# gsalzer/mythril

Hardware: AMD Instinct MI355X
Metric: constraint-candidate evals/sec + % z3 queries discharged on-GPU (higher is better)
Workload: dtype u32 (256-bit as 8x32-bit limbs)

## Files before the change

### mythril_amd/csrc/u256.h

```cpp
#pragma once
#include <math.h>
#include <stdint.h>

#define PF_INL __device__ __forceinline__

#include "u256_cols.h"

namespace pf {

struct u256 {
    uint32_t l[8];
};

PF_INL u256 zero256() {
    u256 r;
#pragma unroll
    for (int i = 0; i < 8; i++) r.l[i] = 0;
    return r;
}

PF_INL u256 ones256() {
    u256 r;
#pragma unroll
    for (int i = 0; i < 8; i++) r.l[i] = 0xffffffffu;
    return r;
}

PF_INL u256 add256(const u256& a, const u256& b) {
    u256 r;
    uint32_t c = 0;
#pragma unroll
    for (int i = 0; i < 8; i++) {
        uint32_t co;
        r.l[i] = __builtin_addc(a.l[i], b.l[i], c, &co);
        c = co;
    }
    return r;
}

PF_INL u256 add256c(const u256& a, const u256& b, uint32_t* cout) {
    u256 r;
    uint32_t c = 0;
#pragma unroll
    for (int i = 0; i < 8; i++) {
        uint32_t co;
        r.l[i] = __builtin_addc(a.l[i], b.l[i], c, &co);
        c = co;
    }
    *cout = c;
    return r;
}

PF_INL u256 sub256(const u256& a, const u256& b) {
    u256 r;
    uint32_t c = 0;
#pragma unroll
    for (int i = 0; i < 8; i++) {
        uint32_t co;
        r.l[i] = __builtin_subc(a.l[i], b.l[i], c, &co);
        c = co;
    }
    return r;
}

PF_INL u256 sub256b(const u256& a, const u256& b, uint32_t* bout) {
    u256 r;
    uint32_t c = 0;
#pragma unroll
    for (int i = 0; i < 8; i++) {
        uint32_t co;
        r.l[i] = __builtin_subc(a.l[i], b.l[i], c, &co);
        c = co;
    }
    *bout = c;
    return r;
}

PF_INL uint32_t ult256(const u256& a, const u256& b) {
    uint32_t c = 0;
#pragma unroll
    for (int i = 0; i < 8; i++) {
        uint32_t co;
        (void)__builtin_subc(a.l[i], b.l[i], c, &co);
        c = co;
    }
    return c;
}

PF_INL uint32_t eq256(const u256& a, const u256& b) {
    uint32_t d = 0;
#pragma unroll
    for (int i = 0; i < 8; i++) d |= a.l[i] ^ b.l[i];
    return d == 0;
}

PF_INL uint32_t iszero256(const u256& a) {
    uint32_t d = 0;
#pragma unroll
    for (int i = 0; i < 8; i++) d |= a.l[i];
    return d == 0;
}

PF_INL u256 neg256(const u256& a) { return sub256(zero256(), a); }

PF_INL u256 not256(const u256& a) {
    u256 r;
#pragma unroll
    for (int i = 0; i < 8; i++) r.l[i] = ~a.l[i];
    return r;
}

PF_INL uint32_t lane_mask(uint32_t c) {
    uint32_t m = 0u - (uint32_t)(c != 0u);
#ifndef PF_HOST_MAC
    asm volatile("" : "+v"(m));
#endif
    return m;
}

PF_INL uint32_t zero_limb() {
    uint32_t z = 0u;
#ifndef PF_HOST_MAC
    asm("" : "+v"(z));
#endif
    return z;
}

PF_INL u256 sel256(uint32_t c, const u256& a, const u256& b) {
    const uint32_t m = lane_mask(c);
    u256 r;
#pragma unroll
    for (int i = 0; i < 8; i++) r.l[i] = (a.l[i] & m) | (b.l[i] & ~m);
    return r;
}

#ifndef PF_HOST_MAC
PF_INL uint32_t wave_max_u32(uint32_t v) {
#pragma unroll
    for (int o = 32; o >= 1; o >>= 1) v = max(v, (uint32_t)__shfl_xor((int)v, o));
    return __builtin_amdgcn_readfirstlane(v);
}
PF_INL uint64_t wave_mask(bool p) { return __builtin_amdgcn_ballot_w64(p); }
#else
PF_INL uint32_t wave_max_u32(uint32_t v) { return v; }
PF_INL uint64_t wave_mask(bool p) { return p ? 1ull : 0ull; }
#endif
PF_INL bool wave_any(uint64_t m) { return m != 0ull; }
PF_INL bool wave_none(uint64_t m) { return m == 0ull; }

PF_INL uint64_t wave_mask_ult256(const u256& a, const u256& b) {
#ifndef PF_HOST_MAC
    uint64_t m;
    uint32_t t;
    asm("v_sub_co_u32 %1, vcc, %2, %10\n\ts_nop 1\n\t"
        "v_subb_co_u32 %1, vcc, %3, %11, vcc\n\ts_nop 1\n\t"
        "v_subb_co_u32 %1, vcc, %4, %12, vcc\n\ts_nop 1\n\t"
        "v_subb_co_u32 %1, vcc, %5, %13, vcc\n\ts_nop 1\n\t"
        "v_subb_co_u32 %1, vcc, %6, %14, vcc\n\ts_nop 1\n\t"
        "v_subb_co_u32 %1, vcc, %7, %15, vcc\n\ts_nop 1\n\t"
        "v_subb_co_u32 %1, vcc, %8, %16, vcc\n\ts_nop 1\n\t"
        "v_subb_co_u32 %1, %0, %9, %17, vcc"
        : "=s"(m), "=&v"(t)
        : "v"(a.l[0]), "v"(a.l[1]), "v"(a.l[2]), "v"(a.l[3]), "v"(a.l[4]), "v"(a.l[5]), "v"(a.l[6]),
          "v"(a.l[7]), "v"(b.l[0]), "v"(b.l[1]), "v"(b.l[2]), "v"(b.l[3]), "v"(b.l[4]), "v"(b.l[5]),
          "v"(b.l[6]), "v"(b.l[7])
        : "vcc");
    return m;
#else
    return wave_mask(ult256(a, b) != 0u);
#endif
}

PF_INL uint32_t sat_u32(double x) {
#ifndef PF_HOST_MAC
    uint32_t r;
    asm("v_cvt_u32_f64 %0, %1" : "=v"(r) : "v"(x));
    return r;
#else
    return (uint32_t)fmin(x, 4294967295.0);
#endif
}

#define PF_COL_NEXT(k)                                   \
    r.l[k] = (uint32_t)acc;                              \
    acc = (acc >> 32) | ((uint64_t)hi << 32);

PF_INL u256 mul256(const u256& a, const u256& b) {
    const uint32_t *x = a.l, *y = b.l;
    u256 r;
    uint64_t acc = 0;
    uint32_t hi = 0;
    col64_1(acc, x[0], y[0]);
    PF_COL_NEXT(0)
    col96_2(acc, hi, x[0], x[1], y[1], y[0]);
    PF_COL_NEXT(1)
    col96_3(acc, hi, x[0], x[1], x[2], y[2], y[1], y[0]);
    PF_COL_NEXT(2)
    col96_4(acc, hi, x[0], x[1], x[2], x[3], y[3], y[2], y[1], y[0]);
    PF_COL_NEXT(3)
    col96_5(acc, hi, x[0], x[1], x[2], x[3], x[4], y[4], y[3], y[2], y[1], y[0]);
    PF_COL_NEXT(4)
    col96_6(acc, hi, x[0], x[1], x[2], x[3], x[4], x[5], y[5], y[4], y[3], y[2], y[1], y[0]);
    PF_COL_NEXT(5)
    col64_7(acc, x[0], x[1], x[2], x[3], x[4], x[5], x[6], y[6], y[5], y[4], y[3], y[2], y[1], y[0]);
    r.l[6] = (uint32_t)acc;
    acc >>= 32;
    col64_8(acc, x[0], x[1], x[2], x[3], x[4], x[5], x[6], x[7], y[7], y[6], y[5], y[4], y[3], y[2], y[1], y[0]);
    r.l[7] = (uint32_t)acc;
    return r;
}

PF_INL u256 sqr256(const u256& a) {
    const uint32_t* x = a.l;
    u256 r;
    r.l[0] = 0u;
    uint64_t acc = 0;
    uint32_t hi = 0;
    col64_1(acc, x[0], x[1]);
    PF_COL_NEXT(1)
    col96_1(acc, hi, x[0], x[2]);
    PF_COL_NEXT(2)
    col96_2(acc, hi, x[0], x[1], x[3], x[2]);
    PF_COL_NEXT(3)
    col96_2(acc, hi, x[0], x[1], x[4], x[3]);
    PF_COL_NEXT(4)
    col96_3(acc, hi, x[0], x[1], x[2], x[5], x[4], x[3]);
    PF_COL_NEXT(5)
    col64_3(acc, x[0], x[1], x[2], x[6], x[5], x[4]);
    r.l[6] = (uint32_t)acc;
    acc >>= 32;
    col64_4(acc, x[0], x[1], x[2], x[3], x[7], x[6], x[5], x[4]);
    r.l[7] = (uint32_t)acc;
    u256 c;
#pragma unroll
    for (int i = 7; i >= 1; i--) c.l[i] = (r.l[i] << 1) | (r.l[i - 1] >> 31);
    c.l[0] = 0u;
    u256 d;
#pragma unroll
    for (int i = 0; i < 4; i++) {
        uint64_t q = 0;
        col64_1(q, x[i], x[i]);
        d.l[2 * i] = (uint32_t)q;
        d.l[2 * i + 1] = (uint32_t)(q >> 32);
    }
    return add256(c, d);
}
#undef PF_COL_NEXT

PF_INL uint32_t mul256_overflows(const u256& a, const u256& b) {
    uint32_t hi = 0;
    u256 r = zero256();
#pragma unroll
    for (int i = 0; i < 8; i++) {
        uint64_t carry = 0;
#pragma unroll
        for (int j = 0; j < 8; j++) {
            if (i + j < 8) {
                uint64_t t = (uint64_t)a.l[i] * b.l[j] + r.l[i + j] + carry;
                r.l[i + j] = (uint32_t)t;
                carry = t >> 32;
            } else {
                hi |= (a.l[i] != 0u && b.l[j] != 0u) ? 1u : 0u;
            }
        }
        hi |= (carry != 0) ? 1u : 0u;
    }
    return hi;
}

PF_INL u256 shl256(const u256& a, uint32_t s, uint32_t big) {
    u256 x = a;
    if (__builtin_expect(1, 1)) {
        uint32_t m = (s >> 7) & 1;
#pragma unroll
        for (int i = 7; i >= 0; i--) x.l[i] = m ? (i >= 4 ? x.l[i - 4] : 0u) : x.l[i];
        m = (s >> 6) & 1;
#pragma unroll
        for (int i = 7; i >= 0; i--) x.l[i] = m ? (i >= 2 ? x.l[i - 2] : 0u) : x.l[i];
        m = (s >> 5) & 1;
#pragma unroll
        for (int i = 7; i >= 0; i--) x.l[i] = m ? (i >= 1 ? x.l[i - 1] : 0u) : x.l[i];
    }
    uint32_t bs = s & 31;
    u256 r;
#pragma unroll
    for (int i = 7; i >= 1; i--) r.l[i] = bs ? ((x.l[i] << bs) | (x.l[i - 1] >> (32 - bs))) : x.l[i];
    r.l[0] = x.l[0] << bs;
    return sel256(big, zero256(), r);
}

PF_INL u256 shr256(const u256& a, uint32_t s, uint32_t f) {
    u256 x = a;
    uint32_t m = (s >> 7) & 1;
#pragma unroll
    for (int i = 0; i < 8; i++) x.l[i] = m ? (i + 4 < 8 ? x.l[i + 4] : f) : x.l[i];
    m = (s >> 6) & 1;
#pragma unroll
    for (int i = 0; i < 8; i++) x.l[i] = m ? (i + 2 < 8 ? x.l[i + 2] : f) : x.l[i];
    m = (s >> 5) & 1;
#pragma unroll
    for (int i = 0; i < 8; i++) x.l[i] = m ? (i + 1 < 8 ? x.l[i + 1] : f) : x.l[i];
    uint32_t bs = s & 31;
    u256 r;
#pragma unroll
    for (int i = 0; i < 7; i++) r.l[i] = bs ? ((x.l[i] >> bs) | (x.l[i + 1] << (32 - bs))) : x.l[i];
    r.l[7] = bs ? ((x.l[7] >> bs) | (f << (32 - bs))) : x.l[7];
    return r;
}

PF_INL uint32_t clz256(const u256& a) {
    uint32_t n = 0, done = 0;
#pragma unroll
    for (int i = 7; i >= 0; i--) {
        uint32_t z = a.l[i] ? (uint32_t)__builtin_clz(a.l[i]) : 32u;
        n += done ? 0u : z;
        done |= (a.l[i] != 0u);
    }
    return n;
}

PF_INL double rcp_f64(double x) {
#ifndef PF_HOST_MAC
    double r = __builtin_amdgcn_rcp(x);
    double e = fma(-x, r, 1.0);
    r = fma(r, e, r);
    e = fma(-x, r, 1.0);
    return fma(r, e, r);
#else
    return 1.0 / x;
#endif
}

PF_INL double to_f64(const u256& a) {
    double d = 0.0;
#pragma unroll
    for (int i = 7; i >= 0; i--) d = fma(d, 4294967296.0, (double)a.l[i]);
    return d;
}

#define PF_DIV_BIAS 0x1p-12
PF_INL void udivrem256(const u256& a, const u256& b, u256* q, u256* r) {
    const uint32_t bz = iszero256(b);
    const uint64_t m_bz = wave_mask(bz != 0u);
#ifndef PF_DIV_FORCE_GENERAL
    if (wave_none(wave_mask(true) & ~(wave_mask_ult256(a, b) | m_bz))) {
        *q = sel256(bz, ones256(), zero256());
        *r = a;
        return;
    }
    if (wave_none(wave_mask((b.l[1] | b.l[2] | b.l[3] | b.l[4] | b.l[5] | b.l[6] | b.l[7]) != 0u))) {
        const uint32_t d = bz ? 1u : b.l[0];
        const double rd = rcp_f64((double)d);
        uint32_t rem = 0;
        u256 Q;
#pragma unroll
        for (int j = 7; j >= 0; j--) {
            const uint64_t num = ((uint64_t)rem << 32) | a.l[j];
            const double dn = (double)rem * 4294967296.0 + (double)a.l[j];
            uint32_t qj = sat_u32(fma(dn, rd, 0x1p-12));
            int64_t rr = (int64_t)(num - (uint64_t)qj * d);
            const uint32_t lo = (uint32_t)(rr < 0);
            qj -= lo;
            rr += (int64_t)(d & lane_mask(lo));
            Q.l[j] = qj;
            rem = (uint32_t)rr;
        }
        u256 R = zero256();
        R.l[0] = rem;
        *q = sel256(bz, ones256(), Q);
        *r = sel256(bz, a, R);
        return;
    }
#endif
    const double rcp = rcp_f64(fmax(to_f64(b), 1.0));
#ifndef PF_DIV_FORCE_GENERAL
    const double qest = fma(to_f64(a), rcp, PF_DIV_BIAS);
    if (wave_none(wave_mask(qest >= 4294967294.0) & ~m_bz)) {
        uint32_t qh = sat_u32(qest);
        u256 R, Q = zero256();
        uint32_t carry = 0, bw = 0;
#pragma unroll
        for (int i = 0; i < 8; i++) {
            const uint64_t p = (uint64_t)qh * b.l[i] + carry;
            carry = (uint32_t)(p >> 32);
            uint32_t bo;
            R.l[i] = __builtin_subc(a.l[i], (uint32_t)p, bw, &bo);
            bw = bo;
        }
        uint32_t bo8;
        const uint32_t r8 = __builtin_subc(zero_limb(), carry, bw, &bo8);
        if (wave_any(wave_mask(r8 != 0u))) {
            const uint32_t neg = (uint32_t)(r8 != 0u);
            const uint32_t m = lane_mask(neg);
            uint32_t c = 0;
#pragma unroll
            for (int i = 0; i < 8; i++) {
                uint32_t co;
                R.l[i] = __builtin_addc(R.l[i], b.l[i] & m, c, &co);
                c = co;
            }
            qh -= neg;
        }
        Q.l[0] = qh;
        *q = sel256(bz, ones256(), Q);
        *r = R;
        return;
    }
#endif
    uint32_t u[9];
#pragma unroll
    for (int i = 0; i < 8; i++) u[i] = a.l[i];
    u256 Q = zero256();
    u[8] = zero_limb();
    uint32_t sfx[9];
    sfx[8] = 0u;
#pragma unroll
    for (int k = 7; k >= 0; k--) sfx[k] = sfx[k + 1] | b.l[k];
#pragma unroll
    for (int j = 7; j >= 0; j--) {
        const uint32_t bhigh = j >= 2 ? sfx[9 - j] : 0u;
        double dr = (double)u[7];
#pragma unroll
        for (int i = 6; i >= j; i--) dr = fma(dr, 4294967296.0, (double)u[i]);
        const double qe = fma(dr, rcp, PF_DIV_BIAS);
        if (wave_none(wave_mask(qe >= 1.0) & ~(m_bz | wave_mask(bhigh != 0u)))) continue;
        const uint32_t skip = bz | (uint32_t)(bhigh != 0u);
        uint32_t q = sat_u32(qe) & ~lane_mask(skip);
        uint64_t carry = 0;
        uint32_t borrow = 0;
#pragma unroll
        for (int i = 0; i + j <= 8; i++) {
            const uint64_t p = (uint64_t)q * (i < 8 ? b.l[i] : 0u) + carry;
            carry = p >> 32;
            uint32_t bo;
            u[j + i] = __builtin_subc(u[j + i], (uint32_t)p, borrow, &bo);
            borrow = bo;
        }
        if (wave_any(wave_mask(u[8] != 0u))) {
            const uint32_t neg = (uint32_t)(u[8] != 0u);
            const uint32_t m = 0u - neg;
            q -= neg;
            uint32_t c = 0;
#pragma unroll
            for (int i = 0; i + j <= 8; i++) {
                uint32_t co;
                u[j + i] = __builtin_addc(u[j + i], (i < 8 ? b.l[i] : 0u) & m, c, &co);
                c = co;
            }
        }
        Q.l[j] = q;
    }
    u256 R;
#pragma unroll
    for (int i = 0; i < 8; i++) R.l[i] = u[i];
    *q = sel256(bz, ones256(), Q);
    *r = R;
}

PF_INL void tbl_put(uint2* tbl, uint32_t stride, uint32_t j, const u256& v) {
#pragma unroll
    for (int p = 0; p < 4; p++) tbl[(j * 4u + p) * stride] = make_uint2(v.l[2 * p], v.l[2 * p + 1]);
}
PF_INL u256 tbl_get(const uint2* tbl, uint32_t stride, uint32_t j) {
    u256 v;
#pragma unroll
    for (int p = 0; p < 4; p++) {
        const uint2 q = tbl[(j * 4u + p) * stride];
        v.l[2 * p] = q.x;
        v.l[2 * p + 1] = q.y;
    }
    return v;
}

template <int WB = 3>
PF_INL u256 exp256(const u256& base, const u256& e, uint32_t nbits, uint2* tbl, uint32_t stride) {
    static_assert(WB >= 1 && WB <= 3, "window");
    constexpr uint32_t NT = 1u << WB;
    u256 r = zero256();
    r.l[0] = 1u;
    if (nbits == 0u) return r;
    tbl_put(tbl, stride, 0u, r);
    tbl_put(tbl, stride, 1u, base);
    if constexpr (WB == 2) {
        const u256 b2 = sqr256(base);
        tbl_put(tbl, stride, 2u, b2);
        tbl_put(tbl, stride, 3u, mul256(b2, base));
    } else {
#pragma unroll 1
        for (uint32_t j = 2; j < NT; j++) {
            const u256 f = tbl_get(tbl, stride, (j & 1u) ? j - 1u : j >> 1);
            const u256 g = (j & 1u) ? base : f;
            tbl_put(tbl, stride, j, mul256(f, g));
        }
    }
    const uint32_t nd = (nbits + WB - 1u) / WB;
    const uint32_t rest = WB * (nd - 1u);
    r = tbl_get(tbl, stride, shr256(e, rest, 0u).l[0] & (NT - 1u));
    u256 ex = shl256(e, (256u - rest) & 255u, 0u);
#pragma unroll 1
    for (uint32_t i = 1; i < nd; i++) {
#pragma unroll 1
        for (int k = 0; k < WB; k++) r = sqr256(r);
        const uint32_t d = ex.l[7] >> (32 - WB);
#pragma unroll
        for (int k = 7; k >= 1; k--) ex.l[k] = (ex.l[k] << WB) | (ex.l[k - 1] >> (32 - WB));
        ex.l[0] <<= WB;
        r = mul256(r, tbl_get(tbl, stride, d));
    }
    return r;
}

template <int WB = 2>
PF_INL u256 exp256_w32(const u256& base, uint32_t e, uint32_t nbits, bool want_b2, uint2* tbl, uint32_t stride) {
    static_assert(WB == 2, "window");
    u256 one = zero256();
    one.l[0] = 1u;
    const bool loop = nbits > 1u;
    if (loop || want_b2) {
        const u256 b2 = sqr256(base);
        tbl_put(tbl, stride, 2u, b2);
        if (loop) {
            tbl_put(tbl, stride, 1u, base);
            tbl_put(tbl, stride, 3u, mul256(b2, base));
        }
    }
    if (!loop) return sel256((uint32_t)(e == 0u), one, base);
    const uint32_t nd = (nbits + WB - 1u) / WB;
    uint32_t d = (e >> (WB * (nd - 1u))) & 3u;
    u256 r = sel256((uint32_t)(d == 0u), one, tbl_get(tbl, stride, d));
#pragma unroll 1
    for (uint32_t i = nd - 1u; i-- > 0u;) {
#pragma unroll 1
        for (int k = 0; k < WB; k++) r = sqr256(r);
        d = (e >> (WB * i)) & 3u;
        r = mul256(r, sel256((uint32_t)(d == 0u), one, tbl_get(tbl, stride, d)));
    }
    return r;
}

#ifndef PF_EXP_SPLIT
#define PF_EXP_SPLIT 8
#endif
#define PF_EXP_WINDOW (PF_EXP_SPLIT <= 20 ? 2 : 3)
#define PF_EXP_TBL_ENTRIES (1 << PF_EXP_WINDOW)

PF_INL uint32_t funnel(uint32_t hi, uint32_t lo, uint32_t s) {
    return (uint32_t)((((uint64_t)hi << 32) | lo) >> s);
}

template <int L>
PF_INL void tsqr(const uint32_t* a, uint32_t* out) {
    uint32_t r[L];
#pragma unroll
    for (int i = 0; i < L; i++) r[i] = 0u;
#pragma unroll
    for (int i = 0; 2 * i + 1 < L; i++) {
        uint64_t c = 0;
#pragma unroll
        for (int j = i + 1; i + j < L; j++) {
            c = (uint64_t)a[i] * a[j] + (uint64_t)r[i + j] + (c >> 32);
            r[i + j] = (uint32_t)c;
        }
    }
#pragma unroll
    for (int i = L - 1; i >= 1; i--) r[i] = funnel(r[i], r[i - 1], 31u);
    r[0] <<= 1;
    uint32_t d[L];
#pragma unroll
    for (int i = 0; 2 * i < L; i++) {
        const uint64_t q = (uint64_t)a[i] * a[i];
        d[2 * i] = (uint32_t)q;
        if (2 * i + 1 < L) d[2 * i + 1] = (uint32_t)(q >> 32);
    }
    uint32_t c = 0;
#pragma unroll
    for (int i = 0; i < L; i++) {
        uint32_t co;
        out[i] = __builtin_addc(r[i], d[i], c, &co);
        c = co;
    }
}

template <int TL, uint32_t TM, int Q>
PF_INL void t_steps(uint32_t* t, uint32_t k0, uint32_t k1) {
    constexpr int L = TL - Q;
#pragma unroll 1
    for (uint32_t k = k0; k < k1; k++) {
        uint32_t sq[L];
        if constexpr (L == 8) {
            u256 a;
#pragma unroll
            for (int i = 0; i < 8; i++) a.l[i] = t[i];
            const u256 s = sqr256(a);
#pragma unroll
            for (int i = 0; i < 8; i++) sq[i] = s.l[i];
        } else {
            tsqr<L>(t, sq);
        }
        const uint32_t sh = 32u - (k + 1u - 32u * Q);
        uint32_t c = 0;
#pragma unroll
        for (int i = Q; i < TL; i++) {
            const uint32_t lo = i > Q ? sq[i > Q ? i - Q - 1 : 0] : 0u;
            uint32_t co;
            t[i] = __builtin_addc(t[i], funnel(sq[i - Q], lo, sh), c, &co);
            c = co;
        }
        t[TL - 1] &= TM;
    }
}


constexpr int v2c(int i) { return (i & 1) ? 0 : 1 + v2c(i >> 1); }
constexpr int v2fact(int j) { return j <= 1 ? 0 : v2c(j) + v2fact(j - 1); }
constexpr int exp_terms(int m) {
    int j = 1;
    while ((j + 1) * (m + 2) - v2fact(j + 1) < 256) j++;
    return j;
}
constexpr int prefix_val(int m, int i) { return (i - 1) * (m + 2) - v2fact(i - 1); }

struct k256 {
    uint32_t l[8];
};
constexpr k256 k_small(uint32_t v) {
    k256 r{};
    r.l[0] = v;
    return r;
}
constexpr k256 k_mul(const k256& a, const k256& b) {
    k256 r{};
    for (int i = 0; i < 8; i++) {
        uint64_t c = 0;
        for (int j = 0; i + j < 8; j++) {
            c = (uint64_t)a.l[i] * b.l[j] + r.l[i + j] + (c >> 32);
            r.l[i + j] = (uint32_t)c;
        }
    }
    return r;
}
constexpr k256 k_inv(const k256& o) {
    k256 x = o;
    for (int it = 0; it < 7; it++) {
        const k256 ox = k_mul(o, x);
        k256 two_minus{};
        uint64_t bw = 0;
        for (int i = 0; i < 8; i++) {
            const uint64_t d = (uint64_t)(i == 0 ? 2u : 0u) - ox.l[i] - bw;
            two_minus.l[i] = (uint32_t)d;
            bw = (d >> 32) & 1u;
        }
        x = k_mul(x, two_minus);
    }
    return x;
}
constexpr k256 exp_oddprod(int i, int j) {
    k256 r = k_small(1u);
    for (int k = i; k <= j; k++) r = k_mul(r, k_small((uint32_t)(k >> v2c(k))));
    return r;
}
constexpr k256 exp_addend(int i, int j, int limbs) {
    k256 r = k_mul(exp_oddprod(i, j), k_inv(exp_oddprod(1, j)));
    for (int k = limbs; k < 8; k++) r.l[k] = 0u;
    return r;
}

template <int L, int LY, uint32_t K0, uint32_t K1, uint32_t K2, uint32_t K3, uint32_t K4, uint32_t K5, uint32_t K6>
PF_INL u256 tmul_add(const u256& a, const u256& b, const k256& k) {
    if constexpr (L >= 8) {
        u256 kk;
#pragma unroll
        for (int i = 0; i < 8; i++) kk.l[i] = k.l[i];
        return add256(mul256(a, b), kk);
    } else {
        u256 r = zero256();
        tmulk<L, LY, K0, K1, K2, K3, K4, K5, K6>(a.l, b.l, r.l);
        return r;
    }
}

template <int L>
PF_INL u256 tmul(const u256& a, const u256& b) {
    if constexpr (L >= 8)
        return mul256(a, b);
    else
        return tmul_add<L, L, 0u, 0u, 0u, 0u, 0u, 0u, 0u>(a, b, k256{});
}

template <int L>
PF_INL u256 sub_mul_small(const u256& a, const u256& b, uint32_t c) {
    u256 r = zero256();
    uint32_t carry = 0, bw = 0;
#pragma unroll
    for (int i = 0; i < L; i++) {
        const uint64_t p = (uint64_t)b.l[i] * c + carry;
        carry = (uint32_t)(p >> 32);
        uint32_t bo;
        r.l[i] = __builtin_subc(a.l[i], (uint32_t)p, bw, &bo);
        bw = bo;
    }
    return r;
}

template <int S, int L>
PF_INL u256 shl_const(const u256& a) {
    constexpr int LS = S / 32, BS = S % 32;
    u256 r = zero256();
#pragma unroll
    for (int i = LS; i < L; i++) {
        const uint32_t hi = a.l[i - LS];
        const uint32_t lo = i - LS - 1 >= 0 ? a.l[i - LS - 1 >= 0 ? i - LS - 1 : 0] : 0u;
        r.l[i] = BS ? funnel(hi, lo, 32 - BS) : hi;
    }
    return r;
}

template <int M, int I, int J>
PF_INL u256 horner(u256& g, const u256& tt) {
    constexpr int S = M + 2 - v2c(I);
    constexpr int P = 256 - prefix_val(M, I);
    constexpr int L = (P + 31) / 32;
    constexpr k256 K = exp_addend(I, J, L);
    constexpr int LY = (I == J || (P - S + 31) / 32 >= L || L == 1) ? L : L - 1;
    u256 inner = zero256();
    if constexpr (I < J) {
        inner = horner<M, I + 1, J>(g, tt);
        g = add256(g, tt);
    } else {
        constexpr k256 C = exp_addend(J + 1, J, L);
#pragma unroll
        for (int i = 0; i < L; i++) inner.l[i] = C.l[i];
    }
    return tmul_add<L, LY, K.l[0], K.l[1], K.l[2], K.l[3], K.l[4], K.l[5], K.l[6]>(shl_const<S, L>(g), inner, K);
}

PF_INL u256 exp256_split(const u256& base, const u256& e, uint2* tbl, uint32_t stride,
                         uint64_t* pt = nullptr) {
#if defined(PF_PROFILE_UNITS) && !defined(PF_HOST_MAC)
#define PF_EXP_STAMP(k)                                        \
    if (pt) {                                                  \
        const uint64_t t_ = __builtin_amdgcn_s_memtime();      \
        pt[k] += t_ - t_last;                                  \
        t_last = t_;                                           \
    }
    uint64_t t_last = __builtin_amdgcn_s_memtime();
#else
#define PF_EXP_STAMP(k)
    (void)pt;
#endif
    constexpr int M = PF_EXP_SPLIT;
    static_assert(M >= 8 && M <= 84, "split");
    constexpr int T = 254 - M;
    constexpr int TL = (T + 31) / 32;
    constexpr uint32_t TM = (T % 32) ? ((1u << (T % 32)) - 1u) : 0xffffffffu;
    constexpr int TB = (T + 3 + 31) / 32;
    constexpr int J = exp_terms(M);
    constexpr int WB = PF_EXP_WINDOW;
    const uint32_t odd = base.l[0] & 1u;
    const uint32_t e_big =
        (e.l[0] >= 256u) | ((e.l[1] | e.l[2] | e.l[3] | e.l[4] | e.l[5] | e.l[6] | e.l[7]) != 0u);
    u256 e0;
#pragma unroll
    for (int i = 0; i < 8; i++)
        e0.l[i] = 32 * i + 32 <= M ? e.l[i] : (32 * i < M ? e.l[i] & ((1u << (M % 32)) - 1u) : 0u);
    const uint32_t nb0 = wave_max_u32(256u - clz256(e0));
    u256 n = shr256(e, (uint32_t)M, 0u);
#pragma unroll
    for (int i = 0; i < 8; i++) n.l[i] = i < TL - 1 ? n.l[i] : (i == TL - 1 ? n.l[i] & TM : 0u);
    const bool series = wave_any(wave_mask(odd != 0u) & ~wave_mask(iszero256(n) != 0u));
    u256 r;
    if constexpr (M <= 32 && WB == 2)
        r = exp256_w32<WB>(base, e0.l[0], nb0 < (uint32_t)M ? nb0 : (uint32_t)M, series && TB == 8, tbl, stride);
    else
        r = exp256<WB>(base, e0, nb0 < (uint32_t)M ? nb0 : (uint32_t)M, tbl, stride);
    PF_EXP_STAMP(0)
    if (series) {
        tbl_put(tbl, stride, 1u, r);
        uint32_t t[TL];
        {
            uint32_t sq[TB];
            if constexpr (M <= 32 && WB == 2 && TB == 8) {
                const u256 b2 = tbl_get(tbl, stride, 2u);
#pragma unroll
                for (int i = 0; i < TB; i++) sq[i] = b2.l[i];
            } else {
                tsqr<TB>(base.l, sq);
            }
            sq[0] -= 1u;
#pragma unroll
            for (int i = 0; i < TL; i++) t[i] = funnel(i + 1 < TB ? sq[i + 1 < TB ? i + 1 : 0] : 0u, sq[i], 3u);
            t[TL - 1] &= TM;
        }
        t_steps<TL, TM, 0>(t, 1u, M < 32 ? (uint32_t)M : 32u);
        if (M > 32) t_steps<TL, TM, 1>(t, 32u, M < 64 ? (uint32_t)M : 64u);
        if (M > 64) t_steps<TL, TM, 2>(t, 64u, (uint32_t)M);
        u256 tt = zero256();
#pragma unroll
        for (int i = 0; i < TL; i++) tt.l[i] = t[i];
        PF_EXP_STAMP(1)
        const u256 nt = tmul<(256 - (M + 2) + 31) / 32>(n, tt);
        u256 g = sub_mul_small<8>(nt, tt, (uint32_t)(J - 1));
        u256 h = horner<M, 1, J>(g, tt);
        u256 one = zero256();
        one.l[0] = 1u;
        h = sel256(odd, h, one);
        r = mul256(tbl_get(tbl, stride, 1u), h);
        PF_EXP_STAMP(2)
    }
    return sel256((odd ^ 1u) & e_big, zero256(), r);
#undef PF_EXP_STAMP
}

}
```

Measured before the change: 7.579 billion.

## Compute series base by full squaring and fold scale shifts into Horner constants

Replaces the truncated incremental t-recurrence (tsqr plus funnel-shift steps) with plain repeated full 256-bit squaring of the base, M times, followed by subtracting one. The Horner evaluation now works on the unshifted G and T, using a constexpr schedule that places the power-of-two scale factors into the shifted addend literals instead of shifting G at every level. This removes the narrower tsqr/t_steps code and the shl_const operations, at the cost of full-width squarings where truncated ones were used before. It also relies on the schedule's static_asserts to keep the scaled values within their limb widths.

Measured after the change: 7.777 billion, median of 6. 1.03x the previous value.

```diff
diff --git a/mythril_amd/csrc/u256.h b/mythril_amd/csrc/u256.h
--- a/mythril_amd/csrc/u256.h
+++ b/mythril_amd/csrc/u256.h
@@ -548,69 +548,6 @@
     return (uint32_t)((((uint64_t)hi << 32) | lo) >> s);
 }
 
-template <int L>
-PF_INL void tsqr(const uint32_t* a, uint32_t* out) {
-    uint32_t r[L];
-#pragma unroll
-    for (int i = 0; i < L; i++) r[i] = 0u;
-#pragma unroll
-    for (int i = 0; 2 * i + 1 < L; i++) {
-        uint64_t c = 0;
-#pragma unroll
-        for (int j = i + 1; i + j < L; j++) {
-            c = (uint64_t)a[i] * a[j] + (uint64_t)r[i + j] + (c >> 32);
-            r[i + j] = (uint32_t)c;
-        }
-    }
-#pragma unroll
-    for (int i = L - 1; i >= 1; i--) r[i] = funnel(r[i], r[i - 1], 31u);
-    r[0] <<= 1;
-    uint32_t d[L];
-#pragma unroll
-    for (int i = 0; 2 * i < L; i++) {
-        const uint64_t q = (uint64_t)a[i] * a[i];
-        d[2 * i] = (uint32_t)q;
-        if (2 * i + 1 < L) d[2 * i + 1] = (uint32_t)(q >> 32);
-    }
-    uint32_t c = 0;
-#pragma unroll
-    for (int i = 0; i < L; i++) {
-        uint32_t co;
-        out[i] = __builtin_addc(r[i], d[i], c, &co);
-        c = co;
-    }
-}
-
-template <int TL, uint32_t TM, int Q>
-PF_INL void t_steps(uint32_t* t, uint32_t k0, uint32_t k1) {
-    constexpr int L = TL - Q;
-#pragma unroll 1
-    for (uint32_t k = k0; k < k1; k++) {
-        uint32_t sq[L];
-        if constexpr (L == 8) {
-            u256 a;
-#pragma unroll
-            for (int i = 0; i < 8; i++) a.l[i] = t[i];
-            const u256 s = sqr256(a);
-#pragma unroll
-            for (int i = 0; i < 8; i++) sq[i] = s.l[i];
-        } else {
-            tsqr<L>(t, sq);
-        }
-        const uint32_t sh = 32u - (k + 1u - 32u * Q);
-        uint32_t c = 0;
-#pragma unroll
-        for (int i = Q; i < TL; i++) {
-            const uint32_t lo = i > Q ? sq[i > Q ? i - Q - 1 : 0] : 0u;
-            uint32_t co;
-            t[i] = __builtin_addc(t[i], funnel(sq[i - Q], lo, sh), c, &co);
-            c = co;
-        }
-        t[TL - 1] &= TM;
-    }
-}
-
-
 constexpr int v2c(int i) { return (i & 1) ? 0 : 1 + v2c(i >> 1); }
 constexpr int v2fact(int j) { return j <= 1 ? 0 : v2c(j) + v2fact(j - 1); }
 constexpr int exp_terms(int m) {
@@ -679,59 +616,105 @@
     }
 }
 
-template <int L>
-PF_INL u256 tmul(const u256& a, const u256& b) {
-    if constexpr (L >= 8)
-        return mul256(a, b);
-    else
-        return tmul_add<L, L, 0u, 0u, 0u, 0u, 0u, 0u, 0u>(a, b, k256{});
-}
-
-template <int L>
-PF_INL u256 sub_mul_small(const u256& a, const u256& b, uint32_t c) {
+PF_INL u256 sub_small256(const u256& a, uint32_t c) {
+    u256 r;
+    uint32_t bw = 0;
+#pragma unroll
+    for (int i = 0; i < 8; i++) {
+        uint32_t bo;
+        r.l[i] = __builtin_subc(a.l[i], i == 0 ? c : 0u, bw, &bo);
+        bw = bo;
+    }
+    return r;
+}
+
+template <int S, int L>
+PF_INL u256 shr_const(const u256& a) {
+    static_assert(S >= 0 && S < 32 && L >= 1 && L <= 8, "shape");
     u256 r = zero256();
-    uint32_t carry = 0, bw = 0;
-#pragma unroll
-    for (int i = 0; i < L; i++) {
-        const uint64_t p = (uint64_t)b.l[i] * c + carry;
-        carry = (uint32_t)(p >> 32);
-        uint32_t bo;
-        r.l[i] = __builtin_subc(a.l[i], (uint32_t)p, bw, &bo);
-        bw = bo;
-    }
-    return r;
-}
-
-template <int S, int L>
-PF_INL u256 shl_const(const u256& a) {
-    constexpr int LS = S / 32, BS = S % 32;
-    u256 r = zero256();
-#pragma unroll
-    for (int i = LS; i < L; i++) {
-        const uint32_t hi = a.l[i - LS];
-        const uint32_t lo = i - LS - 1 >= 0 ? a.l[i - LS - 1 >= 0 ? i - LS - 1 : 0] : 0u;
-        r.l[i] = BS ? funnel(hi, lo, 32 - BS) : hi;
-    }
-    return r;
-}
+#pragma unroll
+    for (int i = 0; i < L; i++) r.l[i] = S ? funnel(i + 1 < 8 ? a.l[i + 1 < 8 ? i + 1 : 0] : 0u, a.l[i], S) : a.l[i];
+    return r;
+}
+
+constexpr k256 k_shl(const k256& k, int s, int limbs) {
+    k256 r{};
+    for (int i = 0; i < limbs; i++) {
+        const uint64_t w = ((uint64_t)k.l[i] << 32) | (i ? k.l[i - 1] : 0u);
+        r.l[i] = (uint32_t)(w >> (32 - s));
+    }
+    return r;
+}
+constexpr bool exp_literal_ok(const k256& k, int limbs) {
+    if (limbs >= 8) return true;
+    for (int c = 2; c < limbs; c++)
+        if (k.l[c] > 0xFFFFFFFFu - (uint32_t)(c - 1)) return false;
+    return true;
+}
+
+constexpr int EXP_MAX_TERMS = 32;
+struct exp_sched_t {
+    int c[EXP_MAX_TERMS + 2];
+    bool unscale[EXP_MAX_TERMS + 2];
+    bool shift_g[EXP_MAX_TERMS + 2];
+};
+constexpr exp_sched_t exp_sched(int m) {
+    exp_sched_t s{};
+    const int j = exp_terms(m);
+    const k256 inv = k_inv(exp_oddprod(1, j));
+    k256 e = k_small(1u);
+    for (int i = j; i >= 1; i--) {
+        e = k_mul(e, k_small((uint32_t)(i >> v2c(i))));
+        const int p = 256 - prefix_val(m, i), l = (p + 31) / 32, v = v2c(i), cin = s.c[i + 1];
+        k256 k = k_mul(e, inv);
+        for (int q = l; q < 8; q++) k.l[q] = 0u;
+        if (p + cin + v <= 32 * l && exp_literal_ok(k_shl(k, cin + v, l), l)) {
+            s.c[i] = cin + v;
+        } else if (p + v <= 32 * l && exp_literal_ok(k_shl(k, v, l), l)) {
+            s.c[i] = v;
+            s.unscale[i] = cin != 0;
+        } else {
+            s.c[i] = 0;
+            s.unscale[i] = cin != 0;
+            s.shift_g[i] = v != 0;
+        }
+    }
+    return s;
+}
+template <int M>
+inline constexpr exp_sched_t EXP_SCHED = exp_sched(M);
 
 template <int M, int I, int J>
-PF_INL u256 horner(u256& g, const u256& tt) {
-    constexpr int S = M + 2 - v2c(I);
+PF_INL u256 horner(u256& G, const u256& T) {
+    static_assert(J <= EXP_MAX_TERMS, "schedule size");
+    constexpr int V = v2c(I);
     constexpr int P = 256 - prefix_val(M, I);
     constexpr int L = (P + 31) / 32;
-    constexpr k256 K = exp_addend(I, J, L);
-    constexpr int LY = (I == J || (P - S + 31) / 32 >= L || L == 1) ? L : L - 1;
+    constexpr int C = EXP_SCHED<M>.c[I];
+    constexpr bool UNSCALE = EXP_SCHED<M>.unscale[I], SHIFT_G = EXP_SCHED<M>.shift_g[I];
+    constexpr int CIN = EXP_SCHED<M>.c[I + 1];
+    constexpr int CY = UNSCALE ? 0 : CIN;
+    static_assert(C == CY + (SHIFT_G ? 0 : V) && C >= 0 && C < 32 && CIN < 32, "scale schedule");
+    static_assert(P + C <= 32 * L, "the scaled level fits its limbs");
+    static_assert(I > 1 || C == 0, "the chain ends unscaled");
+    constexpr k256 K = k_shl(exp_addend(I, J, L), C, L);
+    static_assert(exp_literal_ok(K, L), "shifted addend as column literals");
+    constexpr int PY = P - (M + 2 - V);
+    constexpr int LY = (I == J || (PY + CY + 31) / 32 >= L || L == 1) ? L : L - 1;
     u256 inner = zero256();
     if constexpr (I < J) {
-        inner = horner<M, I + 1, J>(g, tt);
-        g = add256(g, tt);
+        inner = horner<M, I + 1, J>(G, T);
+        G = add256(G, T);
+        if constexpr (UNSCALE) inner = shr_const<CIN, (PY + 31) / 32>(inner);
     } else {
-        constexpr k256 C = exp_addend(J + 1, J, L);
-#pragma unroll
-        for (int i = 0; i < L; i++) inner.l[i] = C.l[i];
-    }
-    return tmul_add<L, LY, K.l[0], K.l[1], K.l[2], K.l[3], K.l[4], K.l[5], K.l[6]>(shl_const<S, L>(g), inner, K);
+        constexpr k256 C0 = exp_addend(J + 1, J, L);
+#pragma unroll
+        for (int i = 0; i < L; i++) inner.l[i] = C0.l[i];
+    }
+    if constexpr (SHIFT_G)
+        return tmul_add<L, LY, K.l[0], K.l[1], K.l[2], K.l[3], K.l[4], K.l[5], K.l[6]>(shr_const<V, L>(G), inner, K);
+    else
+        return tmul_add<L, LY, K.l[0], K.l[1], K.l[2], K.l[3], K.l[4], K.l[5], K.l[6]>(G, inner, K);
 }
 
 PF_INL u256 exp256_split(const u256& base, const u256& e, uint2* tbl, uint32_t stride,
@@ -753,7 +736,6 @@
     constexpr int T = 254 - M;
     constexpr int TL = (T + 31) / 32;
     constexpr uint32_t TM = (T % 32) ? ((1u << (T % 32)) - 1u) : 0xffffffffu;
-    constexpr int TB = (T + 3 + 31) / 32;
     constexpr int J = exp_terms(M);
     constexpr int WB = PF_EXP_WINDOW;
     const uint32_t odd = base.l[0] & 1u;
@@ -770,37 +752,23 @@
     const bool series = wave_any(wave_mask(odd != 0u) & ~wave_mask(iszero256(n) != 0u));
     u256 r;
     if constexpr (M <= 32 && WB == 2)
-        r = exp256_w32<WB>(base, e0.l[0], nb0 < (uint32_t)M ? nb0 : (uint32_t)M, series && TB == 8, tbl, stride);
+        r = exp256_w32<WB>(base, e0.l[0], nb0 < (uint32_t)M ? nb0 : (uint32_t)M, series, tbl, stride);
     else
         r = exp256<WB>(base, e0, nb0 < (uint32_t)M ? nb0 : (uint32_t)M, tbl, stride);
     PF_EXP_STAMP(0)
     if (series) {
         tbl_put(tbl, stride, 1u, r);
-        uint32_t t[TL];
-        {
-            uint32_t sq[TB];
-            if constexpr (M <= 32 && WB == 2 && TB == 8) {
-                const u256 b2 = tbl_get(tbl, stride, 2u);
-#pragma unroll
-                for (int i = 0; i < TB; i++) sq[i] = b2.l[i];
-            } else {
-                tsqr<TB>(base.l, sq);
-            }
-            sq[0] -= 1u;
-#pragma unroll
-            for (int i = 0; i < TL; i++) t[i] = funnel(i + 1 < TB ? sq[i + 1 < TB ? i + 1 : 0] : 0u, sq[i], 3u);
-            t[TL - 1] &= TM;
-        }
-        t_steps<TL, TM, 0>(t, 1u, M < 32 ? (uint32_t)M : 32u);
-        if (M > 32) t_steps<TL, TM, 1>(t, 32u, M < 64 ? (uint32_t)M : 64u);
-        if (M > 64) t_steps<TL, TM, 2>(t, 64u, (uint32_t)M);
-        u256 tt = zero256();
-#pragma unroll
-        for (int i = 0; i < TL; i++) tt.l[i] = t[i];
+        u256 X;
+        if constexpr (M <= 32 && WB == 2)
+            X = tbl_get(tbl, stride, 2u);
+        else
+            X = sqr256(base);
+#pragma unroll 1
+        for (int k = 1; k < M; k++) X = sqr256(X);
+        X.l[0] -= 1u;
         PF_EXP_STAMP(1)
-        const u256 nt = tmul<(256 - (M + 2) + 31) / 32>(n, tt);
-        u256 g = sub_mul_small<8>(nt, tt, (uint32_t)(J - 1));
-        u256 h = horner<M, 1, J>(g, tt);
+        u256 G = mul256(sub_small256(n, (uint32_t)(J - 1)), X);
+        u256 h = horner<M, 1, J>(G, X);
         u256 one = zero256();
         one.l[0] = 1u;
         h = sel256(odd, h, one);
```
